# argriffing/raoteh

Hardware: AMD Instinct MI355X
Metric: site log-likelihoods/sec (batched tree pruning) (higher is better)
Workload: dtype f64; 1 GPU; c3: 61-state MG94 codon, 64-leaf balanced tree, 10000 sites/GPU, dense f64 leaf likelihood vectors; encoding=dense, sites_per_gpu=10000, sites_total=10000, states=61, leaves=64, edges=126, batches_rotated=3, reduce=none

## Files before the change

raoteh_amd/csrc/common.h:

```cpp
#pragma once

#include <hip/hip_runtime.h>
#include <hip/hip_ext.h>

#include <cstdarg>
#include <cstdint>
#include <cstdio>
#include <cstring>
#include <memory>
#include <string>
#include <vector>

#include "../../include/raoteh_hip.h"


void rt_set_error(const char *fmt, ...);

#define RT_HIP(call)                                                          \
    do {                                                                      \
        hipError_t e_ = (call);                                               \
        if (e_ != hipSuccess) {                                               \
            rt_set_error("%s failed: %s (%s:%d)", #call,                      \
                         hipGetErrorString(e_), __FILE__, __LINE__);          \
            return RT_ERR_HIP;                                                \
        }                                                                     \
    } while (0)

#define RT_REQUIRE(cond, ...)                                                 \
    do {                                                                      \
        if (!(cond)) {                                                        \
            rt_set_error(__VA_ARGS__);                                        \
            return RT_ERR_INVALID;                                            \
        }                                                                     \
    } while (0)

#define RT_TRY(call)                                                          \
    do {                                                                      \
        int rc_ = (call);                                                     \
        if (rc_ != RT_OK) return rc_;                                         \
    } while (0)

struct rt_jit_job;


struct rt_timing_slot {
    std::vector<std::pair<hipEvent_t, hipEvent_t>> pending;
    std::vector<hipEvent_t> pool;
    double total_ms = 0.0;
    int64_t launches = 0;
    int64_t seen = 0;
    char name[64] = "";
};

static const int RT_TOTALS_SLOTS = 4096;

struct rt_ctx {
    int device = 0;
    hipStream_t stream = nullptr;
    int num_cus = 0;
    bool timing = false;
    int timing_period = 1;
    rt_timing_slot slots[RT_K_COUNT];
    hipEvent_t ev_start = nullptr, ev_stop = nullptr;
    double *d_totals_arena = nullptr;
    std::vector<int> totals_free;
    hipEvent_t ev_reduced = nullptr;
    hipEvent_t comm_events[8] = {};
    int comm_event_next = 0;
    unsigned char *d_scratch = nullptr;
    size_t scratch_bytes = 0;
    void *comm = nullptr;
    hipStream_t comm_stream = nullptr;
    void *rccl = nullptr;
    int opt_force_generic = -2;
    int opt_jit = -2;
    int opt_jit_block_sites = -2;
    int opt_jit_async = -2;
    int opt_rescale = -2;
    int opt_leaf_state_kernels = -2;
    struct rt_sites *pending_reduce = nullptr;
    size_t expm_attr_lds = 0;
    size_t expm_ts_attr_lds[8] = {0, 0, 0, 0, 0, 0, 0, 0};
    size_t expm_split_attr_lds = 0;
    size_t expm_wide_attr_lds[8] = {0, 0, 0, 0, 0, 0, 0, 0};
    double *d_expm_scratch = nullptr;
    void *expect_cache = nullptr;
    hipStream_t stream2 = nullptr;
    hipEvent_t ev_fork = nullptr, ev_join = nullptr;
    size_t expm_scratch_bytes = 0;
    int live_models = 0, live_chains = 0;
};
static const int RT_OPT_UNSET = -2;

static const int RT_FAST_MAX_DEPTH = 16;

struct rt_op {
    int32_t node;
    int32_t obs;
    int32_t pop;
    int32_t dst;
};

struct rt_model {
    rt_ctx *ctx = nullptr;
    int64_t nnodes = 0;
    int64_t n = 0;
    std::vector<int64_t> indices, indptr;
    std::vector<int32_t> parent;
    std::vector<rt_op> ops;
    std::vector<int32_t> h_qidx;
    std::vector<double> h_t;
    int max_depth = 0;
    int64_t *d_indices = nullptr, *d_indptr = nullptr;
    rt_op *d_ops = nullptr;
    double *d_P = nullptr;
    double *d_Pfrag = nullptr;
    double *d_Pquad = nullptr;
    double *d_Pcol = nullptr;
    double *d_root = nullptr;
    double *d_spec = nullptr;
    bool spectral = false, spectral_has_D = false;
    double *d_Q = nullptr;
    int64_t q_capacity = 0;
    int32_t *d_qidx = nullptr;
    double *d_t = nullptr;
    int32_t *d_info = nullptr;
    int32_t *d_step_of_node = nullptr;
    int32_t *d_qidx_step = nullptr;
    double *d_t_step = nullptr;
    bool have_P = false;
    bool frag_dirty = true;
    int live_batches = 0;
    void *expect_state = nullptr;
    void *expect_lane_state = nullptr;
};

enum { RT_LAYOUT_LANE = 0, RT_LAYOUT_MFMA = 1 };

struct rt_sites {
    rt_model *model = nullptr;
    int64_t nsites = 0;
    int64_t nobs = 0;
    int layout = RT_LAYOUT_LANE;
    bool lane_dma = false;
    int lane_ring = 8;
    bool mfma_solo = false;
    int64_t nblocks = 0;
    int64_t obs_bytes = 0;
    std::vector<int32_t> node_obs;
    std::vector<rt_op> ops;
    rt_op *d_ops = nullptr;
    int32_t *d_lane_ops = nullptr;
    int lane_stack_slots = 1;
    int64_t lane_nprog = 0;
    double *d_obs = nullptr;
    double *d_loglik = nullptr;
    int32_t *d_status = nullptr;
    double *d_partial = nullptr;
    int64_t npartials = 0;
    double *d_totals = nullptr;
    int totals_slot = -1;
    hipEvent_t ev_comm_done = nullptr;
    bool comm_pending = false;
    void *jit_fn = nullptr;
    int jit_prefetch = 0;
    int jit_lookahead = 1;
    int block_sites = 64;
    int jit_waves = 1;
    int jit_tiles = 1;
    void *jit_fn2 = nullptr;
    int jit_tiles2 = 1;
    int64_t jit_split_tiles = 0;
    bool jit_quad = false;
    bool jit_fused = false;
    double *d_partial_alt = nullptr;
    bool jit_halves = false;
    void *jit_combine = nullptr;
    double *d_half = nullptr;
    bool jit_fold = false;
    int *d_half_count = nullptr;
    bool interp_halves = false;
    bool rescale = false;
    int32_t *d_lane_ops_a = nullptr, *d_lane_ops_b = nullptr;
    int32_t *d_down_meta = nullptr;
    int down_slots = 0;
    int half_nops[2] = {0, 0};
    int half_rec1 = 0, half_kobs1 = 0, half_kroot = -1;
    double *d_Lout = nullptr, *d_Mout = nullptr;
    int compact_states = 0;
    double *d_scratch = nullptr;
    int64_t scratch_bytes = 0;
    std::shared_ptr<rt_jit_job> jit_job;
    struct jit_cand { int T; bool halves; bool quad; bool sparse = false; bool pipe = false; };
    std::vector<jit_cand> jit_cands;
    std::vector<std::string> jit_srcs;
    int jit_kind = 0;
    bool keep_raw = false;
    void *d_raw = nullptr;
    int *d_raw_src = nullptr;
    struct { int S = 64, WG = 1, D = 1, LA = 1, compact = 0; bool fuse = false; } jit_lane;
    bool sparse_ok = false;
    bool sparse_pairs = false;
    bool jit_sparse = false;
    bool jit_pipe = false;
    unsigned *d_leafw = nullptr;
    double *d_weights = nullptr;
    unsigned char *d_sets = nullptr;
    rt_sites *expect_twin = nullptr;
    bool obs_borrowed = false;
    bool counted = false;
    bool pruned = false;
    char kernel_name[64] = "";
    double jit_compile_s = 0.0;
};


void rt_time_begin(rt_ctx *ctx, int kernel, const char *name, hipEvent_t *start);
void rt_time_end(rt_ctx *ctx, int kernel, hipEvent_t start);
bool rt_time_extra_begin(rt_ctx *ctx, int kernel, const char *name, hipEvent_t *a, hipEvent_t *b);
void rt_time_extra_end(rt_ctx *ctx, int kernel, hipEvent_t a, hipEvent_t b);

struct rt_reduce_args {
    const double *partial = nullptr;
    long npartials = 0;
    double *totals = nullptr;
    double nsites = 0.0;
};
int rt_expm_wide_launch(rt_ctx *ctx, int nt, bool split2, size_t grid, int64_t n, const double *d_Q,
                        const int *d_qidx, const double *d_t, double *d_P, int *d_info,
                        const int *d_step_of_node, int frag_kind, double *d_Pfrag,
                        const rt_reduce_args &red);
int rt_launch_expm(rt_ctx *ctx, int64_t n, int64_t count, const double *d_Q,
                   const int32_t *d_qidx, const double *d_t, double *d_P,
                   int32_t *d_info, const int32_t *d_step_of_node, int frag_kind,
                   double *d_Pfrag, const rt_reduce_args *fused_reduce = nullptr,
                   double *d_Pquad = nullptr);
// ... 95 lines not shown
```

raoteh_amd/csrc/expm.hip:

```cpp
#include "common.h"

#include <algorithm>
#include "reduce.h"

#include <cstdlib>

namespace {

__constant__ double c_theta[5] = {1.495585217958292e-2, 2.539398330063230e-1,
                                  9.504178996162932e-1, 2.097847961257068e0,
                                  5.371920351148152e0};
__constant__ double c_b3[4] = {120., 60., 12., 1.};
__constant__ double c_b5[6] = {30240., 15120., 3360., 420., 30., 1.};
__constant__ double c_b7[8] = {17297280., 8648640., 1995840., 277200.,
                               25200., 1512., 56., 1.};
__constant__ double c_b9[10] = {17643225600., 8821612800., 2075673600.,
                                302702400., 30270240., 2162160., 110880.,
                                3960., 90., 1.};
__constant__ double c_b13[14] = {64764752532480000., 32382376266240000.,
                                 7771770303897600., 1187353796428800.,
                                 129060195264000., 10559470521600.,
                                 670442572800., 33522128640., 1323241920.,
                                 40840800., 960960., 16380., 182., 1.};

// ... 435 lines not shown
        ap[u] = X + (16 * (rok[u] ? m : 0) + lr) * LD + lq;
        bp[u] = Y + lq * LD + 16 * (cok[u] ? j : 0) + lr;
#pragma unroll
        for (int v = 0; v < RH; ++v) acc[u][v] = (double4_t){0.0, 0.0, 0.0, 0.0};
    }
    if (cf) {
        const double c0 = cf[0], c1 = cf[1], c2 = cf[2];
#pragma unroll
        for (int u = 0; u < RH; ++u)
#pragma unroll
            for (int v = 0; v < RH; ++v)
                if (rok[u] && cok[v]) {
                    const int m = wr * RH + u, j = wc * RH + v;
                    const int col = 16 * j + lr;
#pragma unroll
                    for (int r = 0; r < 4; ++r) {
                        const int row = 16 * m + 4 * r + lq;
                        const int o = row * LD + col;
                        double w = c1 * (R1 ? R1->v[u][v][r] : P1[o]);
                        if (R2) w = fma(c2, R2->v[u][v][r], w);
                        else if (P2) w = fma(c2, P2[o], w);
                        if (row == col && (double)row < cf[3]) w += c0;
                        acc[u][v][r] = w;
                    }
                }
    }
    double a0[RH], b0[RH], a1[RH], b1[RH];
#pragma unroll
    for (int u = 0; u < RH; ++u) {
        a0[u] = ap[u][0];
        b0[u] = bp[u][0];
        a1[u] = ap[u][KS > 1 ? 4 : 0];
        b1[u] = bp[u][KS > 1 ? 4 * LD : 0];
    }
    for (int kk = 0; kk < KS; ++kk) {
        const int kn = kk + 2 < KS ? kk + 2 : KS - 1;
        double a2[RH], b2[RH];
#pragma unroll
        for (int u = 0; u < RH; ++u) { a2[u] = ap[u][4 * kn]; b2[u] = bp[u][4 * kn * LD]; }
        __builtin_amdgcn_sched_barrier(0);
#pragma unroll
        for (int u = 0; u < RH; ++u)
#pragma unroll
            for (int v = 0; v < RH; ++v)
                acc[u][v] = __builtin_amdgcn_mfma_f64_16x16x4f64(a0[u], b0[v], acc[u][v], 0, 0, 0);
        __builtin_amdgcn_sched_barrier(0);
#pragma unroll
        for (int u = 0; u < RH; ++u) { a0[u] = a1[u]; b0[u] = b1[u]; a1[u] = a2[u]; b1[u] = b2[u]; }
    }
    if (out) {
#pragma unroll
        for (int u = 0; u < RH; ++u)
#pragma unroll
            for (int v = 0; v < RH; ++v)
#pragma unroll
                for (int r = 0; r < 4; ++r) out->v[u][v][r] = acc[u][v][r];
    }
    __syncthreads();
#pragma unroll
    for (int u = 0; u < RH; ++u)
#pragma unroll
        for (int v = 0; v < RH; ++v)
            if (rok[u] && cok[v]) {
                const int m = wr * RH + u, j = wc * RH + v;
                const int col = 16 * j + lr;
#pragma unroll
                for (int r = 0; r < 4; ++r) {
                    const int row = 16 * m + 4 * r + lq;
                    C[row * LD + col] = acc[u][v][r];
                    if (top) {
                        double w = top[1] * R1->v[u][v][r];
                        w = fma(top[2], R2->v[u][v][r], w);
                        w = fma(top[3], acc[u][v][r], w);
                        C2[row * LD + col] = w + ((row == col && (double)row < top[4]) ? top[0] : 0.0);
                    }
                }
            }
    __syncthreads();
}

struct half_tiles {
    double v[2][4];
};

__device__ __forceinline__ void load_half_tiles(const double *M, half_tiles &t, int h)
{
    constexpr int LD = 65;
    const int lane = threadIdx.x & 63;
    const int wave = __builtin_amdgcn_readfirstlane(threadIdx.x >> 6);
    const int lr = lane & 15, lq = lane >> 4;
#pragma unroll
    for (int v = 0; v < 2; ++v)
#pragma unroll
        for (int r = 0; r < 4; ++r)
            t.v[v][r] = M[(16 * wave + 4 * r + lq) * LD + 16 * (2 * h + v) + lr];
}

__device__ unsigned long long rt_expm_fine[8];
#define RT_FINE(k) if (fine && threadIdx.x == 0) rt_expm_fine[k] = __builtin_readcyclecounter()

__device__ __forceinline__ void mm_half(const double *X, const double *Y, double *C,
                                        double c0, double c1, double c2, double nd,
                                        const half_tiles &R1, const half_tiles &R2, int h,
                                        bool fine = false)
{
    RT_FINE(0);
    constexpr int LD = 65, KS = 16;
    const int lane = threadIdx.x & 63;
    const int wave = __builtin_amdgcn_readfirstlane(threadIdx.x >> 6);
    const int lr = lane & 15, lq = lane >> 4;
    double4_t acc[2];
    const double *ap = X + (16 * wave + lr) * LD + lq;
    const double *bp = Y + lq * LD + 32 * h + lr;
    double a0 = ap[0], b00 = bp[0], b01 = bp[16];
    double a1 = ap[4], b10 = bp[4 * LD], b11 = bp[4 * LD + 16];
#pragma unroll
    for (int v = 0; v < 2; ++v) {
        const int col = 16 * (2 * h + v) + lr;
#pragma unroll
        for (int r = 0; r < 4; ++r) {
            const int row = 16 * wave + 4 * r + lq;
            double w = c1 * R1.v[v][r];
            w = fma(c2, R2.v[v][r], w);
            if (row == col && (double)row < nd) w += c0;
            acc[v][r] = w;
        }
    }
    RT_FINE(1);
#pragma unroll
    for (int kk = 0; kk < KS; ++kk) {
        const int kn = kk + 2 < KS ? kk + 2 : KS - 1;
        const double a2 = ap[4 * kn], b20 = bp[4 * kn * LD], b21 = bp[4 * kn * LD + 16];
        __builtin_amdgcn_sched_barrier(0);
        acc[0] = __builtin_amdgcn_mfma_f64_16x16x4f64(a0, b00, acc[0], 0, 0, 0);
        acc[1] = __builtin_amdgcn_mfma_f64_16x16x4f64(a0, b01, acc[1], 0, 0, 0);
        __builtin_amdgcn_sched_barrier(0);
        a0 = a1; b00 = b10; b01 = b11;
        a1 = a2; b10 = b20; b11 = b21;
    }
    RT_FINE(2);
    __syncthreads();
    RT_FINE(3);
#pragma unroll
    for (int v = 0; v < 2; ++v) {
        const int col = 16 * (2 * h + v) + lr;
#pragma unroll
        for (int r = 0; r < 4; ++r) C[(16 * wave + 4 * r + lq) * LD + col] = acc[v][r];
    }
    RT_FINE(4);
    __syncthreads();
    RT_FINE(5);
}

__device__ int rt_expm_trace_on = 0;
__device__ unsigned long long rt_expm_trace[8];
#define RT_EXPM_STAMP(k)                                                              \
    if (trace_on && blockIdx.x == (SPLIT ? 2 : 1) && threadIdx.x == 0)                \
        rt_expm_trace[k] = __builtin_readcyclecounter()

template <int NT, bool GLOBAL, bool SPLIT = false>
__global__ void __launch_bounds__(TPB)
expm_taylor_kernel(int n, const double *__restrict__ Q, const int *__restrict__ qidx,
                   const double *__restrict__ tt, double *__restrict__ P,
                   int *__restrict__ info, const int *__restrict__ step_of_node,
                   int frag_kind, double *__restrict__ Pfrag, double *__restrict__ Pquad,
                   double *__restrict__ scratch, rt_reduce_args red)
{
    extern __shared__ __attribute__((aligned(16))) unsigned char smem[];
    if (red.partial && blockIdx.x == gridDim.x - 1) {
        rt_reduce_partials_body(red.partial, red.npartials, red.totals, red.nsites);
        return;
    }
    constexpr int RN = 16 * NT;
    constexpr int LD = RN + 1;
    constexpr int MSZ = RN * LD;
    __shared__ double colsum[RN];
    const int trace_on = rt_expm_trace_on;
    RT_EXPM_STAMP(0);
    double *B0 = GLOBAL ? scratch + (size_t)blockIdx.x * 4 * MSZ : (double *)smem;
    double *B1 = B0 + MSZ;
    double *B2 = B1 + MSZ;
    double *B3 = B2 + MSZ;

    static_assert(!SPLIT || (NT == 4 && !GLOBAL), "two workgroups per matrix: 49 <= n <= 64");
    const int b = SPLIT ? (int)(blockIdx.x >> 1) : (int)blockIdx.x;
    const int half = SPLIT ? (int)(blockIdx.x & 1) : 0;
    const int tid = threadIdx.x;
    const int nn = n * n;
    const int KSn = (n + 3) / 4, NTn = (n + 15) / 16;
    double *Pb = P + (long)b * nn;
    const int qi = qidx[b];
    const int step = step_of_node ? step_of_node[b] : -1;
    constexpr int RP0 = GLOBAL ? 1 : TPB / RN;
    constexpr int PER0 = GLOBAL ? 1 : (RN + RP0 - 1) / RP0;
    double q0[PER0];
    if (!GLOBAL) {
        const int jc = tid % RN, g = tid / RN;
#pragma unroll
        for (int u = 0; u < PER0; ++u) {
            const int i = g + u * RP0;
            q0[u] = (g < RP0 && i < n && jc < n) ? Q[i * n + jc] : 0.0;
        }
    }
    const double t_early = tt[b];
    if (qi < 0) {
        for (int e = tid; e < nn; e += TPB) Pb[e] = 0.0;
        if (info && tid == 0) { info[2 * b] = 0; info[2 * b + 1] = 0; }
        if (step >= 0 && frag_kind == 0)
            for (int e = tid; e < nn; e += TPB) Pfrag[(long)step * nn + e] = 0.0;
        if (step >= 0 && frag_kind == 1) {
            const int total = NTn * ((KSn + 1) / 2) * 128;
            for (int e = tid; e < total; e += TPB) Pfrag[(long)step * total + e] = 0.0;
            if (Pquad)
                for (int e = tid; e < KSn * KSn * 16; e += TPB)
                    Pquad[(long)step * rt_quad_stride(n) + e] = 0.0;
        }
        return;
    }
    const double *Qb = Q + (long)qi * nn;
    const double t = t_early;
    double nrm = 0.0;
    if (!GLOBAL) {
        constexpr int RP = TPB / RN;
        constexpr int PER = (RN + RP - 1) / RP;
        __shared__ double colpart[RP][RN];
        const int jc = tid % RN, g = tid / RN;
        const bool active = g < RP;
        double v[PER];
        double part = 0.0;
        if (qi > 0) {
#pragma unroll
            for (int u = 0; u < PER; ++u) {
                const int i = g + u * RP;
                q0[u] = (active && i < n && jc < n) ? Qb[i * n + jc] : 0.0;
            }
        }
#pragma unroll
        for (int u = 0; u < PER; ++u) v[u] = q0[u] * t;
#pragma unroll
        for (int u = 0; u < PER; ++u) {
            const int i = g + u * RP;
            if (active && i < RN) B0[i * LD + jc] = v[u];
            part += fabs(v[u]);
        }
        if (active) colpart[g][jc] = part;
        __syncthreads();
        if (tid < RN) {
            double sum = 0.0;
#pragma unroll
            for (int r = 0; r < RP; ++r) sum += colpart[r][tid];
            colsum[tid] = sum;
        }
        __syncthreads();
        {
            const int ln = tid & 63;
            nrm = ln < RN ? colsum[ln] : 0.0;
#pragma unroll
            for (int o = 32; o > 0; o >>= 1) nrm = fmax(nrm, __shfl_xor(nrm, o, 64));
        }
    } else {
        constexpr int PER = (MSZ + TPB - 1) / TPB;
        for (int c0 = 0; c0 < PER; c0 += 8) {
            double v[8];
#pragma unroll
            for (int u = 0; u < 8; ++u) {
                const int e = (c0 + u) * TPB + tid;
                const int i = e / LD, jx = e - i * LD;
                v[u] = (e < MSZ && i < n && jx < n) ? Qb[i * n + jx] * t : 0.0;
            }
#pragma unroll
            for (int u = 0; u < 8; ++u) {
                const int e = (c0 + u) * TPB + tid;
                if (e < MSZ) B0[e] = v[u];
            }
        }
        __syncthreads();
        for (int jx = tid; jx < RN; jx += TPB) {
            double sum = 0.0;
            for (int i = 0; i < n; ++i) sum += fabs(B0[i * LD + jx]);
            colsum[jx] = sum;
        }
        __syncthreads();
        for (int jj = 0; jj < RN; ++jj) nrm = fmax(nrm, colsum[jj]);
    }
    RT_EXPM_STAMP(1);
    if (!(nrm < 1e300)) {
        for (int e = tid; e < nn; e += TPB) Pb[e] = __builtin_nan("");
        if (info && tid == 0) { info[2 * b] = -1; info[2 * b + 1] = 0; }
        return;
    }
    int m = 15, s = 0;
    if (nrm <= c_theta_taylor[0]) m = 3;
    else if (nrm <= c_theta_taylor[1]) m = 6;
    else if (nrm <= c_theta_taylor[2]) m = 9;
    else if (nrm <= c_theta_taylor[3]) m = 12;
    else if (nrm > c_theta_taylor[4]) {
        int e;
        const double f = frexp(nrm / c_theta_taylor[4], &e);
        s = (f == 0.5) ? e - 1 : e;
        if (s < 0) s = 0;
    }
    m = __builtin_amdgcn_readfirstlane(m);
    s = __builtin_amdgcn_readfirstlane(s);
    if (info && tid == 0) { info[2 * b] = m; info[2 * b + 1] = s; }
    if (s > 0) {
        const double sc = ldexp(1.0, -s);
        for (int e = tid; e < MSZ; e += TPB) B0[e] *= sc;
        __syncthreads();
    }
    const int q = m / 3;
    RT_EXPM_STAMP(2);
    lane_tiles<NT> ra, ra2;
    load_tiles<NT>(B0, ra);
    mm_blocked<NT>(B0, B0, B1, nullptr, nullptr, nullptr, nullptr, nullptr, &ra2);
    __shared__ double tops[5];
    {
        const int base = 3 * (q - 1);
        if (tid == 0) {
            tops[0] = c_inv_fact[base];
            tops[1] = c_inv_fact[base + 1];
            tops[2] = c_inv_fact[base + 2];
            tops[3] = c_inv_fact[m];
            tops[4] = (double)n;
        }
        __syncthreads();
    }
    mm_blocked<NT>(B0, B1, B2, nullptr, nullptr, nullptr, &ra, &ra2, nullptr, tops, B3);
    RT_EXPM_STAMP(3);
    RT_EXPM_STAMP(4);
    __shared__ double cfs_all[5][4];
    if (tid < 20) cfs_all[tid >> 2][tid & 3] = (tid & 3) == 3 ? (double)n
                                                             : c_inv_fact[3 * (tid >> 2) + (tid & 3)];
    __syncthreads();
    if (SPLIT && s == 0) {
        if constexpr (SPLIT) {
            half_tiles ha, ha2;
            load_half_tiles(B0, ha, half);
            load_half_tiles(B1, ha2, half);
            double hc[4][3];
#pragma unroll
            for (int u = 0; u < 4; ++u)
#pragma unroll
                for (int e = 0; e < 3; ++e) hc[u][e] = c_inv_fact[3 * u + e];
            const double nd = (double)n;
#pragma unroll
            for (int u = 3; u >= 0; --u)
                if (u <= q - 2)
                    mm_half(B2, B3, B3, hc[u][0], hc[u][1], hc[u][2], nd, ha, ha2, half,
                            trace_on && blockIdx.x == 2 && u == 0);
        }
    } else {
        for (int jj = q - 2; jj >= 0; --jj)
            mm_blocked<NT>(B2, B3, B3, cfs_all[jj], B0, B1, &ra, &ra2);
    }
    RT_EXPM_STAMP(5);
    for (int r = 0; r < s; ++r) mm_blocked<NT>(B3, B3, B3, nullptr, nullptr, nullptr);
    RT_EXPM_STAMP(6);

    const double *Xb = B3;
    if constexpr (SPLIT) {
        const int jc = 32 * half + (tid & 31), g = tid >> 5;
        if (jc < n)
            for (int i = g; i < n; i += TPB / 32) Pb[i * n + jc] = Xb[i * LD + jc];
        if (step >= 0 && frag_kind == 1) {
            const int KP = (KSn + 1) / 2;
            const int total = NTn * KP * 128;
            for (int blk = tid >> 7; blk < NTn * 4; blk += TPB >> 7) {
                const int mm = blk >> 2, qq = 4 * half + (blk & 3);
                if (qq < KP) {
                    const int e = (mm * KP + qq) * 128 + (tid & 127);
                    const int e2 = e & 1;
                    const int ln = (e >> 1) & 63;
                    const int row = 16 * mm + (ln & 15);
                    const int col = 4 * (2 * qq + e2) + (ln >> 4);
                    Pfrag[(long)step * total + e] = (col < RN) ? Xb[row * LD + col] : 0.0;
                }
            }
        }
        RT_EXPM_STAMP(7);
        return;
    }
    if (!GLOBAL) {
        constexpr int RP = TPB / RN;
        const int jc = tid % RN, g = tid / RN;
        if (g < RP && jc < n)
            for (int i = g; i < n; i += RP) Pb[i * n + jc] = Xb[i * LD + jc];
    } else {
        for (int e = tid; e < nn; e += TPB) {
            const int i = e / n, j = e - i * n;
            Pb[e] = Xb[i * LD + j];
        }
    }
    if (step >= 0 && frag_kind == 0) {
        for (int e = tid; e < nn; e += TPB) {
            const int i = e / n, j = e - i * n;
            Pfrag[(long)step * nn + e] = Xb[i * LD + j];
        }
    } else if (step >= 0 && frag_kind == 1) {
        const int KP = (KSn + 1) / 2;
        const int total = NTn * KP * 128;
        for (int blk = tid >> 7; blk < NTn * KP; blk += TPB >> 7) {
            const int e = blk * 128 + (tid & 127);
            const int e2 = e & 1;
            const int ln = (e >> 1) & 63;
            const int qq = blk % KP;
            const int mm = blk / KP;
            const int row = 16 * mm + (ln & 15);
            const int col = 4 * (2 * qq + e2) + (ln >> 4);
            Pfrag[(long)step * total + e] = (col < RN) ? Xb[row * LD + col] : 0.0;
        }
        if (Pquad) {
            const int tq = KSn * KSn * 16;
            for (int e = tid; e < tq; e += TPB) {
                const int i = e & 3, k = (e >> 2) & 3, blk = e >> 4;
                const int row = 4 * (blk / KSn) + i, col = 4 * (blk % KSn) + k;
                Pquad[(long)step * rt_quad_stride(n) + e] = Xb[row * LD + col];
            }
        }
    }
    RT_EXPM_STAMP(7);
}


#define RT_SHARED_SOURCE(...) __VA_ARGS__
#include "expm_small.inc"
#undef RT_SHARED_SOURCE

template <int N>
__global__ void __launch_bounds__(256)
expm_small_kernel(int count, const double *__restrict__ Q, const int *__restrict__ qidx,
                  const double *__restrict__ tt, double *__restrict__ P,
                  int *__restrict__ info, const int *__restrict__ step_of_node,
                  double *__restrict__ Pfrag, rt_reduce_args red)
{
    if (red.partial && blockIdx.x == gridDim.x - 1) {
        rt_reduce_partials_body(red.partial, red.npartials, red.totals, red.nsites);
        return;
    }
    const int b = blockIdx.x * 256 + threadIdx.x;
    if (b >= count) return;
    constexpr int NN = N * N;
    double *Pb = P + (long)b * NN;
    const int qi = qidx[b];
    const int step = step_of_node ? step_of_node[b] : -1;
    if (qi < 0) {
#pragma unroll
        for (int e = 0; e < NN; ++e) Pb[e] = 0.0;
        if (info) { info[2 * b] = 0; info[2 * b + 1] = 0; }
        if (step >= 0)
#pragma unroll
            for (int e = 0; e < NN; ++e) Pfrag[(long)step * NN + e] = 0.0;
        return;
    }
    const double *Qb = Q + (long)qi * NN;
    const double t = tt[b];
    SmallMat<N> A;
#pragma unroll
    for (int i = 0; i < N; ++i)
#pragma unroll
        for (int j = 0; j < N; ++j) A.a[i][j] = Qb[i * N + j] * t;
    double nrm = 0.0;
#pragma unroll
    for (int j = 0; j < N; ++j) {
        double cs = 0.0;
#pragma unroll
        for (int i = 0; i < N; ++i) cs += fabs(A.a[i][j]);
        nrm = fmax(nrm, cs);
    }
    int m = 13, s = 0;
    if (nrm <= c_theta[0]) m = 3;
    else if (nrm <= c_theta[1]) m = 5;
    else if (nrm <= c_theta[2]) m = 7;
    else if (nrm <= c_theta[3]) m = 9;
    else if (nrm > c_theta[4]) {
        int e;
        const double f = frexp(nrm / c_theta[4], &e);
        s = (f == 0.5) ? e - 1 : e;
        if (s < 0) s = 0;
    }
    if (info) { info[2 * b] = m; info[2 * b + 1] = s; }
    if (s > 0) {
        const double sc = ldexp(1.0, -s);
#pragma unroll
        for (int i = 0; i < N; ++i)
#pragma unroll
            for (int j = 0; j < N; ++j) A.a[i][j] *= sc;
    }
    SmallMat<N> A2, A4, A6, U, V, W, Z;
    sm_comb(Z, 0.0, A, 0.0, A, 0.0, A, 0.0);
    sm_mul(A, A, A2);
    A4 = Z; A6 = Z;
    if (m >= 5) sm_mul(A2, A2, A4);
    if (m >= 7) sm_mul(A4, A2, A6);
    if (m == 13) {
        sm_comb(W, c_b13[13], A6, c_b13[11], A4, c_b13[9], A2, 0.0);
        sm_mul(A6, W, W);
        sm_comb(U, c_b13[7], A6, c_b13[5], A4, c_b13[3], A2, c_b13[1]);
        sm_comb(W, 1.0, W, 1.0, U, 0.0, Z, 0.0);
        sm_mul(A, W, U);
        sm_comb(W, c_b13[12], A6, c_b13[10], A4, c_b13[8], A2, 0.0);
        sm_mul(A6, W, W);
        sm_comb(V, c_b13[6], A6, c_b13[4], A4, c_b13[2], A2, c_b13[0]);
        sm_comb(V, 1.0, V, 1.0, W, 0.0, Z, 0.0);
    } else {
        SmallMat<N> A8 = Z;
        if (m >= 9) sm_mul(A6, A2, A8);
        const double *bc = (m == 3) ? c_b3 : (m == 5) ? c_b5 : (m == 7) ? c_b7 : c_b9;
        const double b5 = m >= 5 ? bc[5] : 0.0, b4 = m >= 5 ? bc[4] : 0.0;
        const double b7 = m >= 7 ? bc[7] : 0.0, b6 = m >= 7 ? bc[6] : 0.0;
        const double b9 = m >= 9 ? bc[9] : 0.0, b8 = m >= 9 ? bc[8] : 0.0;
        sm_comb(W, bc[3], A2, b5, A4, b7, A6, bc[1]);
        sm_comb(W, 1.0, W, b9, A8, 0.0, Z, 0.0);
        sm_comb(V, bc[2], A2, b4, A4, b6, A6, bc[0]);
        sm_comb(V, 1.0, V, b8, A8, 0.0, Z, 0.0);
        sm_mul(A, W, U);
    }
    SmallMat<N> M, X;
    sm_comb(M, 1.0, V, -1.0, U, 0.0, Z, 0.0);
    sm_comb(X, 1.0, V, 1.0, U, 0.0, Z, 0.0);
    bool singular = false;
#pragma unroll
    for (int k = 0; k < N; ++k) {
#pragma unroll
        for (int i = k + 1; i < N; ++i) {
            const bool sw = fabs(M.a[i][k]) > fabs(M.a[k][k]);
#pragma unroll
            for (int j = 0; j < N; ++j) {
                const double mk = M.a[k][j], mi = M.a[i][j];
                M.a[k][j] = sw ? mi : mk;
                M.a[i][j] = sw ? mk : mi;
                const double xk = X.a[k][j], xi = X.a[i][j];
                X.a[k][j] = sw ? xi : xk;
                X.a[i][j] = sw ? xk : xi;
            }
        }
        singular |= !(fabs(M.a[k][k]) > 0.0);
        const double rinv = 1.0 / M.a[k][k];
#pragma unroll
        for (int i = k + 1; i < N; ++i) {
            const double f = M.a[i][k] * rinv;
#pragma unroll
            for (int j = k + 1; j < N; ++j) M.a[i][j] = fma(-f, M.a[k][j], M.a[i][j]);
#pragma unroll
            for (int j = 0; j < N; ++j) X.a[i][j] = fma(-f, X.a[k][j], X.a[i][j]);
        }
    }
#pragma unroll
    for (int k = N - 1; k >= 0; --k) {
        const double rinv = 1.0 / M.a[k][k];
#pragma unroll
        for (int j = 0; j < N; ++j) {
            double acc = X.a[k][j];
#pragma unroll
            for (int i = k + 1; i < N; ++i) acc = fma(-M.a[k][i], X.a[i][j], acc);
            X.a[k][j] = acc * rinv;
        }
    }
    for (int q = 0; q < s; ++q) sm_mul(X, X, X);
    if (singular) {
        if (info) info[2 * b] = -1;
#pragma unroll
        for (int i = 0; i < N; ++i)
#pragma unroll
            for (int j = 0; j < N; ++j) X.a[i][j] = __builtin_nan("");
    }
#pragma unroll
// ... 24 lines not shown
    const int step = step_of_node ? step_of_node[b] : -1;
    const double t = tt[b];
    SmallMat<N> A;
#pragma unroll
    for (int i = 0; i < N; ++i)
#pragma unroll
        for (int j = 0; j < N; ++j) A.a[i][j] = Q[i * N + j];
    if (qi < 0) {
#pragma unroll
        for (int e = 0; e < NN; ++e) Pb[e] = 0.0;
        if (info) { info[2 * b] = 0; info[2 * b + 1] = 0; }
        if (step >= 0)
#pragma unroll
            for (int e = 0; e < NN; ++e) Pfrag[(long)step * NN + e] = 0.0;
        return;
    }
    if (qi > 0) {
        const double *Qb = Q + (long)qi * NN;
#pragma unroll
        for (int i = 0; i < N; ++i)
#pragma unroll
            for (int j = 0; j < N; ++j) A.a[i][j] = Qb[i * N + j];
    }
#pragma unroll
    for (int i = 0; i < N; ++i)
#pragma unroll
        for (int j = 0; j < N; ++j) A.a[i][j] *= t;
    SmallMat<N> X;
    int m, s;
    rt_expm_small_taylor<N>(A, X, m, s);
    if (info) { info[2 * b] = m; info[2 * b + 1] = s; }
#pragma unroll
    for (int i = 0; i < N; ++i)
#pragma unroll
        for (int j = 0; j < N; ++j) {
            Pb[i * N + j] = X.a[i][j];
            if (step >= 0) Pfrag[(long)step * NN + i * N + j] = X.a[i][j];
        }
}

}

int rt_launch_expm(rt_ctx *ctx, int64_t n, int64_t count, const double *d_Q,
                   const int32_t *d_qidx, const double *d_t, double *d_P,
                   int32_t *d_info, const int32_t *d_step_of_node, int frag_kind,
                   double *d_Pfrag, const rt_reduce_args *fused_reduce, double *d_Pquad)
{
    const rt_reduce_args red = fused_reduce ? *fused_reduce : rt_reduce_args();
    const unsigned extra = red.partial ? 1u : 0u;
    if (n < 1 || n > RT_MAX_EXPM_STATES) {
        rt_set_error("expm: n=%lld outside 1..%d", (long long)n, RT_MAX_EXPM_STATES);
        return RT_ERR_UNSUPPORTED;
    }
    const int64_t RT_MAX_PADE_STATES = 62;
    if (count <= 0 && !extra) return RT_OK;
    const int ld = (int)n | 1;
    const size_t lds = (size_t)5 * n * ld * 8 + (128 + 128 + 64) * 8 + (8 + 64) * 4;
    size_t &attr_lds = ctx->expm_attr_lds;
    if (n <= RT_MAX_PADE_STATES && lds > attr_lds) {
        RT_HIP(hipFuncSetAttribute((const void *)expm_kernel,
                                   hipFuncAttributeMaxDynamicSharedMemorySize,
                                   (int)lds));
        attr_lds = lds;
    }
    if (n <= 4 && !getenv("RAOTEH_EXPM_NO_SMALL")) {
        hipEvent_t ev = nullptr;
        const char *wh = getenv("RAOTEH_EXPM");
        const bool pade = wh && strcmp(wh, "pade") == 0;
        rt_time_begin(ctx, RT_K_EXPM, pade ? "expm_small_lane_per_matrix_pade"
                                           : "expm_small_lane_per_matrix", &ev);
        const unsigned grid = (unsigned)((count + 255) / 256) + extra;
        const int *son = frag_kind == 0 ? d_step_of_node : nullptr;
        if (!pade) {
#define RT_SMALLT(NV)                                                                \
            RT_LAUNCH_TIMED(ctx, expm_small_taylor_kernel<NV>, dim3(grid), dim3(256), 0, \
                            (int)count, d_Q, d_qidx, d_t, d_P, d_info, son, d_Pfrag, red)
            switch ((int)n) {
            case 1: RT_SMALLT(1); break;
            case 2: RT_SMALLT(2); break;
            case 3: RT_SMALLT(3); break;
            default: RT_SMALLT(4); break;
            }
#undef RT_SMALLT
            RT_HIP(hipGetLastError());
            rt_time_end(ctx, RT_K_EXPM, ev);
            return RT_OK;
        }
#define RT_SMALL(NV)                                                                 \
        RT_LAUNCH_TIMED(ctx, expm_small_kernel<NV>, dim3(grid), dim3(256), 0, \
                           (int)count, d_Q, d_qidx, d_t, d_P, d_info, son, d_Pfrag, red)
        switch ((int)n) {
        case 1: RT_SMALL(1); break;
        case 2: RT_SMALL(2); break;
        case 3: RT_SMALL(3); break;
        default: RT_SMALL(4); break;
        }
#undef RT_SMALL
        RT_HIP(hipGetLastError());
        rt_time_end(ctx, RT_K_EXPM, ev);
        return RT_OK;
    }
    const char *which = getenv("RAOTEH_EXPM");
    if (n > RT_MAX_PADE_STATES || !(which && strcmp(which, "pade") == 0)) {
        const int nt = (int)((n + 15) / 16);
        const size_t msz = (size_t)(16 * nt) * (16 * nt + 1);
        const bool global = nt > 4;
        const size_t lds_t = global ? 0 : 4 * msz * 8;
        double *scratch = nullptr;
        if (global) {
            const size_t need = (size_t)count * 4 * msz * 8;
            if (need > ctx->expm_scratch_bytes) {
                RT_HIP(hipStreamSynchronize(ctx->stream));
                hipFree(ctx->d_expm_scratch);
                ctx->d_expm_scratch = nullptr;
                ctx->expm_scratch_bytes = 0;
                RT_HIP(hipMalloc((void **)&ctx->d_expm_scratch, need));
                ctx->expm_scratch_bytes = need;
            }
            scratch = ctx->d_expm_scratch;
        }
        const char *wv = getenv("RAOTEH_EXPM_WIDE");
        if (global && !(wv && atoi(wv) == 0) && !d_Pquad) {
            bool split2 = 2 * count + extra <= (int64_t)std::max(2, ctx->num_cus);
            if (const char *v = getenv("RAOTEH_EXPM_SPLIT")) split2 = atoi(v) != 0;
            const size_t wgs = (size_t)count * (split2 ? 2 : 1);
            const size_t need = wgs * ((nt + 1) / 2) * 4 * nt * 256 * 8;
            if (need > ctx->expm_scratch_bytes) {
                RT_HIP(hipStreamSynchronize(ctx->stream));
                hipFree(ctx->d_expm_scratch);
                ctx->d_expm_scratch = nullptr;
                ctx->expm_scratch_bytes = 0;
                RT_HIP(hipMalloc((void **)&ctx->d_expm_scratch, need));
                ctx->expm_scratch_bytes = need;
            }
            RT_TRY(rt_expm_wide_launch(ctx, nt, split2, wgs + extra, n, d_Q, d_qidx, d_t, d_P, d_info,
                                       d_step_of_node, frag_kind, d_Pfrag, red));
            return RT_OK;
        }
        hipEvent_t ev = nullptr;
        rt_time_begin(ctx, RT_K_EXPM, global ? "expm_taylor_ps_mfma_global" : "expm_taylor_ps_mfma",
                      &ev);
#define RT_TAYLOR(NTV, GL)                                                                      \
        do {                                                                                    \
            if (lds_t > ctx->expm_ts_attr_lds[NTV - 1]) {                                       \
                RT_HIP(hipFuncSetAttribute((const void *)expm_taylor_kernel<NTV, GL>,           \
                                           hipFuncAttributeMaxDynamicSharedMemorySize,          \
                                           (int)lds_t));                                        \
                ctx->expm_ts_attr_lds[NTV - 1] = lds_t;                                         \
            }                                                                                   \
            RT_LAUNCH_TIMED(ctx, (expm_taylor_kernel<NTV, GL>), dim3((unsigned)count + extra),  \
                            dim3(TPB), lds_t, (int)n, d_Q, d_qidx, d_t, d_P, d_info,            \
                            d_step_of_node, frag_kind, d_Pfrag, d_Pquad, scratch, red);         \
        } while (0)
        bool split2 = nt == 4 && 2 * count + extra <= (int64_t)std::max(2, ctx->num_cus) && !d_Pquad;
        if (const char *v = getenv("RAOTEH_EXPM_SPLIT")) split2 = nt == 4 && !d_Pquad && atoi(v) != 0;
        if (split2) {
            if (lds_t > ctx->expm_split_attr_lds) {
                RT_HIP(hipFuncSetAttribute((const void *)expm_taylor_kernel<4, false, true>,
                                           hipFuncAttributeMaxDynamicSharedMemorySize, (int)lds_t));
                ctx->expm_split_attr_lds = lds_t;
            }
            snprintf(ctx->slots[RT_K_EXPM].name, sizeof(ctx->slots[RT_K_EXPM].name),
                     "expm_taylor_ps_mfma_split2");
            RT_LAUNCH_TIMED(ctx, (expm_taylor_kernel<4, false, true>),
                            dim3(2u * (unsigned)count + extra), dim3(TPB), lds_t, (int)n, d_Q, d_qidx,
                            d_t, d_P, d_info, d_step_of_node, frag_kind, d_Pfrag, d_Pquad, scratch,
                            red);
        } else
        switch (nt) {
        case 1: RT_TAYLOR(1, false); break;
        case 2: RT_TAYLOR(2, false); break;
        case 3: RT_TAYLOR(3, false); break;
        case 4: RT_TAYLOR(4, false); break;
        case 5: RT_TAYLOR(5, true); break;
        case 6: RT_TAYLOR(6, true); break;
        case 7: RT_TAYLOR(7, true); break;
        default: RT_TAYLOR(8, true); break;
        }
#undef RT_TAYLOR
        RT_HIP(hipGetLastError());
        if (getenv("RAOTEH_EXPM_TRACE")) {
            static int armed = 0;
            unsigned long long tr[8];
            RT_HIP(hipStreamSynchronize(ctx->stream));
            if (armed) {
                RT_HIP(hipMemcpyFromSymbol(tr, HIP_SYMBOL(rt_expm_trace), sizeof tr));
                unsigned long long fn[8];
                RT_HIP(hipMemcpyFromSymbol(fn, HIP_SYMBOL(rt_expm_fine), sizeof fn));
                fprintf(stderr, "[raoteh_amd] last Horner half product: seed + first operands %llu, k loop "
                        "%llu, barrier %llu, write-back %llu, barrier %llu\n", fn[1] - fn[0],
                        fn[2] - fn[1], fn[3] - fn[2], fn[4] - fn[3], fn[5] - fn[4]);
                fprintf(stderr, "[raoteh_amd] expm trace (clocks, workgroup 1): load + norm %llu, order %llu, "
                        "A^2 A^3 %llu, block %llu, Horner %llu, squarings %llu, store %llu; total %llu\n",
                        tr[1] - tr[0], tr[2] - tr[1], tr[3] - tr[2], tr[4] - tr[3], tr[5] - tr[4],
                        tr[6] - tr[5], tr[7] - tr[6], tr[7] - tr[0]);
            }
            const int on = 1;
            RT_HIP(hipMemcpyToSymbol(HIP_SYMBOL(rt_expm_trace_on), &on, sizeof on));
            armed = 1;
        }
        rt_time_end(ctx, RT_K_EXPM, ev);
        return RT_OK;
    }
    hipEvent_t ev = nullptr;
    rt_time_begin(ctx, RT_K_EXPM, "expm_mfma_regsolve", &ev);
    RT_LAUNCH_TIMED(ctx, expm_kernel, dim3((unsigned)count + extra), dim3(TPB), lds,
                       (int)n, d_Q, d_qidx, d_t, d_P, d_info, d_step_of_node, frag_kind,
                       d_Pfrag, d_Pquad, red);
    RT_HIP(hipGetLastError());
    rt_time_end(ctx, RT_K_EXPM, ev);
    return RT_OK;
}
```

Before: 50.70 million sites/s.

## Run expm Taylor kernel with eight waves per workgroup for 33-64 states

Adds an 8-wave (512-thread) variant of the LDS-resident expm Taylor kernel for NT=3/4, with a new per-wave tile assignment so each wave computes fewer MFMA output tiles per matrix product. It aims to put two waves on each SIMD to hide LDS and MFMA latency in the matrix products that compute transition matrices. It is enabled by default for 61-state codon models and can be turned off with RAOTEH_EXPM_WAVES=4. The cost is more barrier participants, uneven tiles for NT=3, and possibly tighter register limits.

```diff
diff --git a/raoteh_amd/csrc/common.h b/raoteh_amd/csrc/common.h
--- a/raoteh_amd/csrc/common.h
+++ b/raoteh_amd/csrc/common.h
@@ -82,6 +82,7 @@
     size_t expm_attr_lds = 0;
     size_t expm_ts_attr_lds[8] = {0, 0, 0, 0, 0, 0, 0, 0};
     size_t expm_split_attr_lds = 0;
+    size_t expm_w8_attr_lds[3] = {0, 0, 0};
     size_t expm_wide_attr_lds[8] = {0, 0, 0, 0, 0, 0, 0, 0};
     double *d_expm_scratch = nullptr;
     void *expect_cache = nullptr;
diff --git a/raoteh_amd/csrc/expm.hip b/raoteh_amd/csrc/expm.hip
--- a/raoteh_amd/csrc/expm.hip
+++ b/raoteh_amd/csrc/expm.hip
@@ -611,14 +611,121 @@
     RT_FINE(5);
 }
 
+template <int NT>
+__device__ __forceinline__ void wave8_tiles(int wave, int &m, int &j0, int &nc)
+{
+    if (NT == 4) { m = wave >> 1; j0 = 2 * (wave & 1); nc = 2; }
+    else if (wave < 6) { m = wave / 3; j0 = wave - 3 * m; nc = 1; }
+    else { m = 2; j0 = wave == 6 ? 0 : 2; nc = wave == 6 ? 2 : 1; }
+}
+
+template <int NT>
+__device__ __forceinline__ void load_left8(const double *X, int m, double (&a)[4 * NT])
+{
+    constexpr int LD = 16 * NT + 1;
+    const int lane = threadIdx.x & 63;
+    const double *ap = X + (16 * m + (lane & 15)) * LD + (lane >> 4);
+#pragma unroll
+    for (int kk = 0; kk < 4 * NT; ++kk) a[kk] = ap[4 * kk];
+}
+
+template <int NT>
+__device__ __forceinline__ void load_tiles8(const double *M, half_tiles &t, int m, int j0, int nc)
+{
+    constexpr int LD = 16 * NT + 1;
+    const int lane = threadIdx.x & 63;
+    const int lr = lane & 15, lq = lane >> 4;
+#pragma unroll
+    for (int v = 0; v < 2; ++v)
+#pragma unroll
+        for (int r = 0; r < 4; ++r)
+            t.v[v][r] = v < nc ? M[(16 * m + 4 * r + lq) * LD + 16 * (j0 + v) + lr] : 0.0;
+}
+
+template <int NT, int NC>
+__device__ __forceinline__ void mm8(const double (&a)[4 * NT], const double *Y, double *C,
+                                    int m, int j0, int nc_wave, bool seed, double c0, double c1,
+                                    double c2, double nd, const half_tiles *R1,
+                                    const half_tiles *R2, half_tiles *out = nullptr,
+                                    const double *top = nullptr, double *C2 = nullptr,
+                                    bool fine = false)
+{
+    RT_FINE(0);
+    constexpr int LD = 16 * NT + 1, KS = 4 * NT;
+    const int nc = NC ? NC : nc_wave;
+    const int lane = threadIdx.x & 63;
+    const int lr = lane & 15, lq = lane >> 4;
+    const double *bp = Y + lq * LD + 16 * j0 + lr;
+    const int o1 = nc > 1 ? 16 : 0;
+    double b00 = bp[0], b01 = bp[o1];
+    double b10 = bp[4 * LD], b11 = bp[4 * LD + o1];
+    double4_t acc[2];
+#pragma unroll
+    for (int v = 0; v < 2; ++v) {
+        acc[v] = (double4_t){0.0, 0.0, 0.0, 0.0};
+        if (seed && v < nc) {
+            const int col = 16 * (j0 + v) + lr;
+#pragma unroll
+            for (int r = 0; r < 4; ++r) {
+                const int row = 16 * m + 4 * r + lq;
+                double w = c1 * R1->v[v][r];
+                w = fma(c2, R2->v[v][r], w);
+                if (row == col && (double)row < nd) w += c0;
+                acc[v][r] = w;
+            }
+        }
+    }
+    RT_FINE(1);
+#pragma unroll
+    for (int kk = 0; kk < KS; ++kk) {
+        const int kn = kk + 2 < KS ? kk + 2 : KS - 1;
+        const double b20 = bp[4 * kn * LD], b21 = bp[4 * kn * LD + o1];
+        __builtin_amdgcn_sched_barrier(0);
+        acc[0] = __builtin_amdgcn_mfma_f64_16x16x4f64(a[kk], b00, acc[0], 0, 0, 0);
+        if (NC != 1 && nc > 1)
+            acc[1] = __builtin_amdgcn_mfma_f64_16x16x4f64(a[kk], b01, acc[1], 0, 0, 0);
+        __builtin_amdgcn_sched_barrier(0);
+        b00 = b10; b01 = b11;
+        b10 = b20; b11 = b21;
+    }
+    RT_FINE(2);
+    if (out) {
+#pragma unroll
+        for (int v = 0; v < 2; ++v)
+#pragma unroll
+            for (int r = 0; r < 4; ++r) out->v[v][r] = acc[v][r];
+    }
+    __syncthreads();
+    RT_FINE(3);
+#pragma unroll
+    for (int v = 0; v < 2; ++v)
+        if (v < nc) {
+            const int col = 16 * (j0 + v) + lr;
+#pragma unroll
+            for (int r = 0; r < 4; ++r) {
+                const int row = 16 * m + 4 * r + lq;
+                C[row * LD + col] = acc[v][r];
+                if (top) {
+                    double w = top[1] * R1->v[v][r];
+                    w = fma(top[2], R2->v[v][r], w);
+                    w = fma(top[3], acc[v][r], w);
+                    C2[row * LD + col] = w + ((row == col && (double)row < top[4]) ? top[0] : 0.0);
+                }
+            }
+        }
+    RT_FINE(4);
+    __syncthreads();
+    RT_FINE(5);
+}
+
 __device__ int rt_expm_trace_on = 0;
 __device__ unsigned long long rt_expm_trace[8];
 #define RT_EXPM_STAMP(k)                                                              \
     if (trace_on && blockIdx.x == (SPLIT ? 2 : 1) && threadIdx.x == 0)                \
         rt_expm_trace[k] = __builtin_readcyclecounter()
 
-template <int NT, bool GLOBAL, bool SPLIT = false>
-__global__ void __launch_bounds__(TPB)
+template <int NT, bool GLOBAL, bool SPLIT = false, int WAVES = 4>
+__global__ void __launch_bounds__(64 * WAVES)
 expm_taylor_kernel(int n, const double *__restrict__ Q, const int *__restrict__ qidx,
                    const double *__restrict__ tt, double *__restrict__ P,
                    int *__restrict__ info, const int *__restrict__ step_of_node,
@@ -642,6 +749,9 @@
     double *B3 = B2 + MSZ;
 
     static_assert(!SPLIT || (NT == 4 && !GLOBAL), "two workgroups per matrix: 49 <= n <= 64");
+    static_assert(WAVES == 4 || (WAVES == 8 && !GLOBAL && (NT == 3 || NT == 4)),
+                  "two waves per SIMD: LDS-resident, 33 <= n <= 64");
+    constexpr int NTH = 64 * WAVES;
     const int b = SPLIT ? (int)(blockIdx.x >> 1) : (int)blockIdx.x;
     const int half = SPLIT ? (int)(blockIdx.x & 1) : 0;
     const int tid = threadIdx.x;
@@ -663,15 +773,15 @@
     }
     const double t_early = tt[b];
     if (qi < 0) {
-        for (int e = tid; e < nn; e += TPB) Pb[e] = 0.0;
+        for (int e = tid; e < nn; e += NTH) Pb[e] = 0.0;
         if (info && tid == 0) { info[2 * b] = 0; info[2 * b + 1] = 0; }
         if (step >= 0 && frag_kind == 0)
-            for (int e = tid; e < nn; e += TPB) Pfrag[(long)step * nn + e] = 0.0;
+            for (int e = tid; e < nn; e += NTH) Pfrag[(long)step * nn + e] = 0.0;
         if (step >= 0 && frag_kind == 1) {
             const int total = NTn * ((KSn + 1) / 2) * 128;
-            for (int e = tid; e < total; e += TPB) Pfrag[(long)step * total + e] = 0.0;
+            for (int e = tid; e < total; e += NTH) Pfrag[(long)step * total + e] = 0.0;
             if (Pquad)
-                for (int e = tid; e < KSn * KSn * 16; e += TPB)
+                for (int e = tid; e < KSn * KSn * 16; e += NTH)
                     Pquad[(long)step * rt_quad_stride(n) + e] = 0.0;
         }
         return;
@@ -744,7 +854,7 @@
     }
     RT_EXPM_STAMP(1);
     if (!(nrm < 1e300)) {
-        for (int e = tid; e < nn; e += TPB) Pb[e] = __builtin_nan("");
+        for (int e = tid; e < nn; e += NTH) Pb[e] = __builtin_nan("");
         if (info && tid == 0) { info[2 * b] = -1; info[2 * b + 1] = 0; }
         return;
     }
@@ -764,67 +874,112 @@
     if (info && tid == 0) { info[2 * b] = m; info[2 * b + 1] = s; }
     if (s > 0) {
         const double sc = ldexp(1.0, -s);
-        for (int e = tid; e < MSZ; e += TPB) B0[e] *= sc;
+        for (int e = tid; e < MSZ; e += NTH) B0[e] *= sc;
         __syncthreads();
     }
     const int q = m / 3;
     RT_EXPM_STAMP(2);
-    lane_tiles<NT> ra, ra2;
-    load_tiles<NT>(B0, ra);
-    mm_blocked<NT>(B0, B0, B1, nullptr, nullptr, nullptr, nullptr, nullptr, &ra2);
-    __shared__ double tops[5];
-    {
-        const int base = 3 * (q - 1);
-        if (tid == 0) {
-            tops[0] = c_inv_fact[base];
-            tops[1] = c_inv_fact[base + 1];
-            tops[2] = c_inv_fact[base + 2];
-            tops[3] = c_inv_fact[m];
-            tops[4] = (double)n;
-        }
+    if constexpr (WAVES == 8) {
+        const int wave = __builtin_amdgcn_readfirstlane(tid >> 6);
+        int wm, wj, wn;
+        wave8_tiles<NT>(wave, wm, wj, wn);
+        constexpr int NCF = NT == 4 ? 2 : 0;
+        const double nd = (double)n;
+        const double tops8[5] = {c_inv_fact[3 * (q - 1)], c_inv_fact[3 * (q - 1) + 1],
+                                 c_inv_fact[3 * (q - 1) + 2], c_inv_fact[m], nd};
+        double left[4 * NT];
+        half_tiles ra, ra2;
+        load_left8<NT>(B0, wm, left);
+        load_tiles8<NT>(B0, ra, wm, wj, wn);
+        mm8<NT, NCF>(left, B0, B1, wm, wj, wn, false, 0.0, 0.0, 0.0, nd, nullptr, nullptr,
+                     &ra2);
+        mm8<NT, NCF>(left, B1, B2, wm, wj, wn, false, 0.0, 0.0, 0.0, nd, &ra, &ra2, nullptr,
+                     tops8, B3);
+        RT_EXPM_STAMP(3);
+        RT_EXPM_STAMP(4);
+        if (q >= 2) load_left8<NT>(B2, wm, left);
+        if (SPLIT && s == 0) {
+            if constexpr (SPLIT) {
+                const int hj = 2 * half + (wave & 1);
+                half_tiles ha, ha2;
+                load_tiles8<NT>(B0, ha, wm, hj, 1);
+                load_tiles8<NT>(B1, ha2, wm, hj, 1);
+#pragma unroll
+                for (int u = 3; u >= 0; --u)
+                    if (u <= q - 2)
+                        mm8<NT, 1>(left, B3, B3, wm, hj, 1, true, c_inv_fact[3 * u],
+                                   c_inv_fact[3 * u + 1], c_inv_fact[3 * u + 2], nd, &ha, &ha2,
+                                   nullptr, nullptr, nullptr,
+                                   trace_on && blockIdx.x == 2 && u == 0);
+            }
+        } else {
+            for (int jj = q - 2; jj >= 0; --jj)
+                mm8<NT, NCF>(left, B3, B3, wm, wj, wn, true, c_inv_fact[3 * jj],
+                             c_inv_fact[3 * jj + 1], c_inv_fact[3 * jj + 2], nd, &ra, &ra2);
+        }
+        RT_EXPM_STAMP(5);
+        for (int r = 0; r < s; ++r) {
+            load_left8<NT>(B3, wm, left);
+            mm8<NT, NCF>(left, B3, B3, wm, wj, wn, false, 0.0, 0.0, 0.0, nd, nullptr, nullptr);
+        }
+    } else {
+        lane_tiles<NT> ra, ra2;
+        load_tiles<NT>(B0, ra);
+        mm_blocked<NT>(B0, B0, B1, nullptr, nullptr, nullptr, nullptr, nullptr, &ra2);
+        __shared__ double tops[5];
+        {
+            const int base = 3 * (q - 1);
+            if (tid == 0) {
+                tops[0] = c_inv_fact[base];
+                tops[1] = c_inv_fact[base + 1];
+                tops[2] = c_inv_fact[base + 2];
+                tops[3] = c_inv_fact[m];
+                tops[4] = (double)n;
+            }
+            __syncthreads();
+        }
+        mm_blocked<NT>(B0, B1, B2, nullptr, nullptr, nullptr, &ra, &ra2, nullptr, tops, B3);
+        RT_EXPM_STAMP(3);
+        RT_EXPM_STAMP(4);
+        __shared__ double cfs_all[5][4];
+        if (tid < 20) cfs_all[tid >> 2][tid & 3] = (tid & 3) == 3 ? (double)n
+                                                                 : c_inv_fact[3 * (tid >> 2) + (tid & 3)];
         __syncthreads();
-    }
-    mm_blocked<NT>(B0, B1, B2, nullptr, nullptr, nullptr, &ra, &ra2, nullptr, tops, B3);
-    RT_EXPM_STAMP(3);
-    RT_EXPM_STAMP(4);
-    __shared__ double cfs_all[5][4];
-    if (tid < 20) cfs_all[tid >> 2][tid & 3] = (tid & 3) == 3 ? (double)n
-                                                             : c_inv_fact[3 * (tid >> 2) + (tid & 3)];
-    __syncthreads();
-    if (SPLIT && s == 0) {
-        if constexpr (SPLIT) {
-            half_tiles ha, ha2;
-            load_half_tiles(B0, ha, half);
-            load_half_tiles(B1, ha2, half);
-            double hc[4][3];
-#pragma unroll
-            for (int u = 0; u < 4; ++u)
-#pragma unroll
-                for (int e = 0; e < 3; ++e) hc[u][e] = c_inv_fact[3 * u + e];
-            const double nd = (double)n;
-#pragma unroll
-            for (int u = 3; u >= 0; --u)
-                if (u <= q - 2)
-                    mm_half(B2, B3, B3, hc[u][0], hc[u][1], hc[u][2], nd, ha, ha2, half,
-                            trace_on && blockIdx.x == 2 && u == 0);
-        }
-    } else {
-        for (int jj = q - 2; jj >= 0; --jj)
-            mm_blocked<NT>(B2, B3, B3, cfs_all[jj], B0, B1, &ra, &ra2);
-    }
-    RT_EXPM_STAMP(5);
-    for (int r = 0; r < s; ++r) mm_blocked<NT>(B3, B3, B3, nullptr, nullptr, nullptr);
+        if (SPLIT && s == 0) {
+            if constexpr (SPLIT) {
+                half_tiles ha, ha2;
+                load_half_tiles(B0, ha, half);
+                load_half_tiles(B1, ha2, half);
+                double hc[4][3];
+#pragma unroll
+                for (int u = 0; u < 4; ++u)
+#pragma unroll
+                    for (int e = 0; e < 3; ++e) hc[u][e] = c_inv_fact[3 * u + e];
+                const double nd = (double)n;
+#pragma unroll
+                for (int u = 3; u >= 0; --u)
+                    if (u <= q - 2)
+                        mm_half(B2, B3, B3, hc[u][0], hc[u][1], hc[u][2], nd, ha, ha2, half,
+                                trace_on && blockIdx.x == 2 && u == 0);
+            }
+        } else {
+            for (int jj = q - 2; jj >= 0; --jj)
+                mm_blocked<NT>(B2, B3, B3, cfs_all[jj], B0, B1, &ra, &ra2);
+        }
+        RT_EXPM_STAMP(5);
+        for (int r = 0; r < s; ++r) mm_blocked<NT>(B3, B3, B3, nullptr, nullptr, nullptr);
+    }
     RT_EXPM_STAMP(6);
 
     const double *Xb = B3;
     if constexpr (SPLIT) {
         const int jc = 32 * half + (tid & 31), g = tid >> 5;
         if (jc < n)
-            for (int i = g; i < n; i += TPB / 32) Pb[i * n + jc] = Xb[i * LD + jc];
+            for (int i = g; i < n; i += NTH / 32) Pb[i * n + jc] = Xb[i * LD + jc];
         if (step >= 0 && frag_kind == 1) {
             const int KP = (KSn + 1) / 2;
             const int total = NTn * KP * 128;
-            for (int blk = tid >> 7; blk < NTn * 4; blk += TPB >> 7) {
+            for (int blk = tid >> 7; blk < NTn * 4; blk += NTH >> 7) {
                 const int mm = blk >> 2, qq = 4 * half + (blk & 3);
                 if (qq < KP) {
                     const int e = (mm * KP + qq) * 128 + (tid & 127);
@@ -840,7 +995,7 @@
         return;
     }
     if (!GLOBAL) {
-        constexpr int RP = TPB / RN;
+        constexpr int RP = NTH / RN;
         const int jc = tid % RN, g = tid / RN;
         if (g < RP && jc < n)
             for (int i = g; i < n; i += RP) Pb[i * n + jc] = Xb[i * LD + jc];
@@ -851,14 +1006,14 @@
         }
     }
     if (step >= 0 && frag_kind == 0) {
-        for (int e = tid; e < nn; e += TPB) {
+        for (int e = tid; e < nn; e += NTH) {
             const int i = e / n, j = e - i * n;
             Pfrag[(long)step * nn + e] = Xb[i * LD + j];
         }
     } else if (step >= 0 && frag_kind == 1) {
         const int KP = (KSn + 1) / 2;
         const int total = NTn * KP * 128;
-        for (int blk = tid >> 7; blk < NTn * KP; blk += TPB >> 7) {
+        for (int blk = tid >> 7; blk < NTn * KP; blk += NTH >> 7) {
             const int e = blk * 128 + (tid & 127);
             const int e2 = e & 1;
             const int ln = (e >> 1) & 63;
@@ -870,7 +1025,7 @@
         }
         if (Pquad) {
             const int tq = KSn * KSn * 16;
-            for (int e = tid; e < tq; e += TPB) {
+            for (int e = tid; e < tq; e += NTH) {
                 const int i = e & 3, k = (e >> 2) & 3, blk = e >> 4;
                 const int row = 4 * (blk / KSn) + i, col = 4 * (blk % KSn) + k;
                 Pquad[(long)step * rt_quad_stride(n) + e] = Xb[row * LD + col];
@@ -1201,9 +1356,28 @@
                             dim3(TPB), lds_t, (int)n, d_Q, d_qidx, d_t, d_P, d_info,            \
                             d_step_of_node, frag_kind, d_Pfrag, d_Pquad, scratch, red);         \
         } while (0)
+#define RT_TAYLOR8(NTV, SP, SLOT)                                                               \
+        do {                                                                                    \
+            if (lds_t > ctx->expm_w8_attr_lds[SLOT]) {                                          \
+                RT_HIP(hipFuncSetAttribute((const void *)expm_taylor_kernel<NTV, false, SP, 8>, \
+                                           hipFuncAttributeMaxDynamicSharedMemorySize,          \
+                                           (int)lds_t));                                        \
+                ctx->expm_w8_attr_lds[SLOT] = lds_t;                                            \
+            }                                                                                   \
+            RT_LAUNCH_TIMED(ctx, (expm_taylor_kernel<NTV, false, SP, 8>),                       \
+                            dim3((SP ? 2u : 1u) * (unsigned)count + extra), dim3(512), lds_t,   \
+                            (int)n, d_Q, d_qidx, d_t, d_P, d_info, d_step_of_node, frag_kind,   \
+                            d_Pfrag, d_Pquad, scratch, red);                                    \
+        } while (0)
+        const char *wv8 = getenv("RAOTEH_EXPM_WAVES");
+        const bool waves8 = (nt == 3 || nt == 4) && !(wv8 && atoi(wv8) == 4);
         bool split2 = nt == 4 && 2 * count + extra <= (int64_t)std::max(2, ctx->num_cus) && !d_Pquad;
         if (const char *v = getenv("RAOTEH_EXPM_SPLIT")) split2 = nt == 4 && !d_Pquad && atoi(v) != 0;
-        if (split2) {
+        if (split2 && waves8) {
+            snprintf(ctx->slots[RT_K_EXPM].name, sizeof(ctx->slots[RT_K_EXPM].name),
+                     "expm_taylor_ps_mfma_split2");
+            RT_TAYLOR8(4, true, 2);
+        } else if (split2) {
             if (lds_t > ctx->expm_split_attr_lds) {
                 RT_HIP(hipFuncSetAttribute((const void *)expm_taylor_kernel<4, false, true>,
                                            hipFuncAttributeMaxDynamicSharedMemorySize, (int)lds_t));
@@ -1219,14 +1393,15 @@
         switch (nt) {
         case 1: RT_TAYLOR(1, false); break;
         case 2: RT_TAYLOR(2, false); break;
-        case 3: RT_TAYLOR(3, false); break;
-        case 4: RT_TAYLOR(4, false); break;
+        case 3: if (waves8) RT_TAYLOR8(3, false, 0); else RT_TAYLOR(3, false); break;
+        case 4: if (waves8) RT_TAYLOR8(4, false, 1); else RT_TAYLOR(4, false); break;
         case 5: RT_TAYLOR(5, true); break;
         case 6: RT_TAYLOR(6, true); break;
         case 7: RT_TAYLOR(7, true); break;
         default: RT_TAYLOR(8, true); break;
         }
 #undef RT_TAYLOR
+#undef RT_TAYLOR8
         RT_HIP(hipGetLastError());
         if (getenv("RAOTEH_EXPM_TRACE")) {
             static int armed = 0;
```

Measured after the change: 51.50 million sites/s (median of 6 runs). 1.02x the previous value.
